# mikestir/webradio

Measured on AMD Instinct MI355X. Metric: complex Msamples/sec (node), 256-ch DDC+NFM demod, higher is better.
Workload: dtype f32

## Files before the change

include/webradio_amd.h:

```cpp
#ifndef WEBRADIO_AMD_H_
#define WEBRADIO_AMD_H_

#include <stddef.h>
#include <stdint.h>

#ifdef __cplusplus
extern "C" {
#endif

#define WR_ABI_VERSION   6
#define WR_FIR_LENGTH    64
#define WR_TABLE_SIZE    65536

enum wr_status {
	WR_OK = 0,
	WR_ERR_ARG = 1,
	WR_ERR_HIP = 2,
	WR_ERR_STATE = 3,
	WR_ERR_NOMEM = 4,
	WR_ERR_NODEV = 5,
	WR_ERR_RATE = 6
};

enum wr_mode { WR_AM = 0, WR_FM = 1, WR_USB = 2, WR_LSB = 3 };
// ... 128 lines not shown
int wr_tuner_mark_launches(wr_tuner *tuner, int enable);
int wr_ring_exchange_after(wr_ring *ring, wr_tuner *tuner, const float *send_dev, float *recv_dev, size_t nfloats);
int wr_ring_wait(wr_ring *ring);
int wr_ring_info(wr_ring *ring, int *rank, int *world, unsigned long long *exchanges);
int wr_ring_destroy(wr_ring *ring);
int wr_tuner_set_audio_scale(wr_tuner *tuner, float scale);

int wr_tuner_set_blocks_per_launch(wr_tuner *tuner, unsigned int nblocks);

#define WR_STREAM_MAX_BLOCKS 512u
int wr_tuner_set_streaming(wr_tuner *tuner, int enable);
int wr_tuner_stream_info(wr_tuner *tuner, int *live, unsigned long long *launches, unsigned long long *blocks);
int wr_tuner_stream_host_blocks(wr_tuner *tuner, unsigned long long *blocks);
int wr_tuner_stream_long_blocks(wr_tuner *tuner, unsigned long long *blocks);

int wr_tuner_profile(wr_tuner *tuner, int enable);
int wr_tuner_profile_read(wr_tuner *tuner, unsigned int *launches, double *mean_ms);

int wr_spectrum_create(wr_spectrum **spec, wr_dev *dev, unsigned int fft_size, unsigned int hop);
int wr_spectrum_create_real(wr_spectrum **spec, wr_dev *dev, unsigned int fft_size, unsigned int hop);
int wr_spectrum_channels(wr_spectrum *spec, unsigned int *channels);
int wr_spectrum_destroy(wr_spectrum *spec);
int wr_spectrum_push(wr_spectrum *spec, const float *iq, size_t nframes, int where);
int wr_spectrum_lazy_info(wr_spectrum *spec, unsigned long long *deferred_pushes, unsigned long long *resolves);
int wr_spectrum_get_db(wr_spectrum *spec, float *magnitudes_host );
int wr_spectrum_get_bins(wr_spectrum *spec, float *bins_host );
int wr_spectrum_frames_done(wr_spectrum *spec, unsigned long *frames);
int wr_spectrum_get_waterfall_row(wr_spectrum *spec, unsigned int width, int hold,
                                  float *db_row_host, uint8_t *palette_host);
int wr_spectrum_batch_db(wr_spectrum *spec, const float *iq_dev, size_t nframes_fft,
// ... 9 lines not shown
```

webradio_amd/capi.py:

```python
import ctypes as C
import os

_HERE = os.path.dirname(os.path.abspath(__file__))
LIB_PATH = os.path.join(_HERE, "lib", "libwebradio_amd.so")

WR_OK, WR_ERR_ARG, WR_ERR_HIP, WR_ERR_STATE, WR_ERR_NOMEM, WR_ERR_NODEV, WR_ERR_RATE = range(7)
WR_AM, WR_FM, WR_USB, WR_LSB = range(4)
WR_STAGE_CHAN_IQ, WR_STAGE_DEMOD, WR_STAGE_AUDIO = 1, 2, 3
WR_NCO_SPLIT, WR_NCO_EXACT, WR_NCO_ROTATE = 0, 1, 2
WR_HOST, WR_DEVICE = 0, 1
WR_ABI_VERSION = 6
WR_STREAM_MAX_BLOCKS = 512
WR_FIR_LENGTH = 64
WR_TABLE_SIZE = 65536

_fp = C.POINTER(C.c_float)
_vp = C.c_void_p
_u32 = C.c_uint
_sz = C.c_size_t

SIGNATURES = {
    "wr_abi_version": (C.c_int, []),
    "wr_last_error": (C.c_char_p, []),
    "wr_device_count": (C.c_int, [C.POINTER(C.c_int)]),
# ... 32 lines not shown
    "wr_chan_set_if": (C.c_int, [_vp, C.c_int, C.c_int]),
    "wr_chan_set_filter": (C.c_int, [_vp, C.c_int, C.c_int, _u32, _u32]),
    "wr_chan_set_taps": (C.c_int, [_vp, C.c_int, C.c_int, _vp, _u32]),
    "wr_chan_set_filter_n": (C.c_int, [_vp, C.c_int, C.c_int, _u32, _u32, _u32]),
    "wr_chan_set_taps_n": (C.c_int, [_vp, C.c_int, C.c_int, _vp, _u32, _u32]),
    "wr_chan_set_mode": (C.c_int, [_vp, C.c_int, C.c_int]),
    "wr_chan_set_af_gain": (C.c_int, [_vp, C.c_int, C.c_float]),
    "wr_chan_set_squelch": (C.c_int, [_vp, C.c_int, C.c_float, C.c_int]),
    "wr_tuner_keep_stages": (C.c_int, [_vp, _u32]),
    "wr_tuner_flush": (C.c_int, [_vp]),
    "wr_tuner_set_blocks_per_launch": (C.c_int, [_vp, _u32]),
    "wr_tuner_set_streaming": (C.c_int, [_vp, C.c_int]),
    "wr_tuner_stream_info": (C.c_int, [_vp, C.POINTER(C.c_int), C.POINTER(C.c_ulonglong), C.POINTER(C.c_ulonglong)]),
    "wr_tuner_stream_host_blocks": (C.c_int, [_vp, C.POINTER(C.c_ulonglong)]),
    "wr_tuner_stream_long_blocks": (C.c_int, [_vp, C.POINTER(C.c_ulonglong)]),
    "wr_tuner_seek": (C.c_int, [_vp, C.c_ulonglong]),
    "wr_tuner_audio_ring": (C.c_int, [_vp, _u32]),
    "wr_tuner_audio_ring_acquire": (C.c_int, [_vp, C.POINTER(C.POINTER(C.c_float)), C.POINTER(C.c_size_t),
                                              C.POINTER(C.c_size_t), C.POINTER(_u32), C.POINTER(C.c_ulonglong)]),
    "wr_tuner_audio_ring_release": (C.c_int, [_vp]),
    "wr_tuner_audio_ring_ready": (C.c_int, [_vp, C.POINTER(C.c_int)]),
    "wr_tuner_audio_ring_stats": (C.c_int, [_vp, C.POINTER(_u32), C.POINTER(C.c_ulonglong)]),
    "wr_tuner_submit_count": (C.c_int, [_vp, C.POINTER(C.c_ulonglong)]),
    "wr_chan_get_state": (C.c_int, [_vp, C.c_int, C.POINTER(_u32), _vp]),
    "wr_chan_set_state": (C.c_int, [_vp, C.c_int, _u32, _vp]),
    "wr_tuner_submit": (C.c_int, [_vp, _vp, _sz, C.c_int]),
    "wr_tuner_last_staging": (C.c_int, [_vp, C.POINTER(C.c_int)]),
    "wr_block_kernel_calls": (C.c_ulonglong, []),
    "wr_tuner_submit_u8": (C.c_int, [_vp, _vp, _sz, C.c_int]),
    "wr_chan_fetch": (C.c_int, [_vp, C.c_int, C.c_int, _vp, _sz, C.POINTER(_sz)]),
# ... 77 lines not shown
```

webradio_amd/csrc/wr_capi_internal.h:

```cpp
#ifndef WR_CAPI_INTERNAL_H
#define WR_CAPI_INTERNAL_H

#include "wr_internal.h"

#include <cstdarg>
#include <cstdio>
#include <cstdlib>
#include <cstring>
#include <new>
#include <atomic>
#include <chrono>
#include <map>
#include <mutex>
#include <vector>

#define HIP_TRY(expr)                                                                    \
	do {                                                                                 \
		hipError_t e_ = (expr);                                                          \
		if (e_ != hipSuccess)                                                            \
			return wrc_fail(WR_ERR_HIP, "%s: %s (%s:%d)", #expr, hipGetErrorString(e_),  \
			                __FILE__, __LINE__);                                         \
	} while (0)


// ... 72 lines not shown
	bool seek_pending = false;
	unsigned long long seek_frame = 0;
	float *z_hist = nullptr, *z_prev = nullptr, *z_dem = nullptr;
	bool pend_direct = false;
	unsigned long long pend_seq = 0;
	size_t pend_k2 = 0;
	unsigned int pend_slots = 0;
	int sp;
	int cb;
	int last_cb;
	std::vector<int> owner;
	bool dirty;
	bool uniform_taps;
	unsigned long long uniform_mask = 0;
	unsigned long long uniform2_mask = 0;
	unsigned long long fewsets_mask = 0;
	unsigned char nsets[64] = {0};
	bool one_filter = false;
	bool long_uniform = false;
	bool long_one = false;
	size_t last_k1, last_k2;
	int active;
};

struct wr_tuner {
	wr_dev *dev;
	unsigned int input_rate;
	unsigned int max_channels;
	size_t max_block_frames;
	int nco_mode;
// ... 46 lines not shown
		bool host_bytes = false;
		bool live = false;
		bool unchecked = false;
		WrStreamCtl *ctl = nullptr;
		WrStreamDesc *desc = nullptr;
		WrStreamDev *sdev = nullptr;
		float *ring = nullptr;
		size_t ring_floats = 0;
		Group *g = nullptr;
		unsigned int count = 0;
		size_t nframes = 0;
		bool u8 = false;
		int parity0 = 0;
		size_t k1 = 0, k2 = 0;
		unsigned long long gen = 0;
		unsigned long long blocks = 0;
		std::chrono::steady_clock::time_point last_bell;
		const float *last_iq = nullptr;
		uint8_t *raw[4] = {nullptr, nullptr, nullptr, nullptr};
		size_t raw_cap = 0;
		unsigned long long raw_next = 0;
		unsigned long long raw_gen[4] = {0, 0, 0, 0};
		unsigned int raw_idx[4] = {0, 0, 0, 0};
		hipEvent_t raw_ev = nullptr;
		bool ext = false;
		bool up_pending = false;
		unsigned long long host_blocks = 0;
		unsigned long long long_blocks = 0;
	} stream;
};
// ... 65 lines not shown
```

webradio_amd/csrc/wr_internal.h:

```cpp
#ifndef WR_INTERNAL_H_
#define WR_INTERNAL_H_

#include <hip/hip_runtime.h>
#include <stddef.h>
#include <stdint.h>

#include "webradio_amd.h"

#define WR_HIST      (WR_FIR_LENGTH - 1)
#define WR_LANES     64
#define WR_SPLIT_N   256
#define WR_MAX_DEVICES 64
#define WR_TAPSETS   4

int         wrc_fail(int code, const char *fmt, ...) __attribute__((format(printf, 2, 3)));
int         wrc_dev_index(const wr_dev *dev);
hipStream_t wrc_dev_stream(const wr_dev *dev);
int         wrc_tuner_launch_mark(wr_tuner *t, hipEvent_t *ev);

void     wrd_sin_table(float *table);
void     wrd_sin_table_rounded(float *table);
int      wrd_phase_step(int if_hz, unsigned int input_rate);
unsigned wrd_lowpass_maxbin(unsigned int fir_length, unsigned int passband, unsigned int input_rate);
void     wrd_lowpass_design(unsigned int fir_length, unsigned int passband, unsigned int input_rate, float *coeff);
// ... 36 lines not shown
	float       *hist_next;
	int          parity;
	int          sp;
	int          cb;
	size_t       nframes;
	unsigned int d1, d2;
	unsigned int slots;
	unsigned int slots_used;
	size_t       k1, k2;
	size_t       k2max;
	int          nco_mode;
	float        audio_scale;
	int          use_gain, use_squelch;
	unsigned long long uniform_mask;
	unsigned long long uniform2_mask;
	unsigned long long fewsets_mask;
	unsigned char nsets[64];
	int          one_filter;
	void        *ev_start, *ev_stop;
	bool         seeking = false;
	unsigned int seek_lo = 0;
};

hipError_t wrk_mix(hipStream_t st, const float *in, float *out, size_t nframes,
                   unsigned int phase, int step, const float *table_dev);
hipError_t wrk_fir(hipStream_t st, const float *in, size_t nframes, unsigned int channels,
                   unsigned int decim, unsigned int fir_length, const float *coeff_dev, const float *hist_dev,
                   float *out);
hipError_t wrk_hist_update(hipStream_t st, const float *in, size_t nframes, unsigned int channels,
                           unsigned int fir_length, float *hist_dev, float *scratch_dev);
// ... 6 lines not shown
struct WrPostArgs {
	const float *chan_iq;
	unsigned int k1, slots;
	const int   *mode;
	const float *prev_iq;
	float       *prev_next;
	const float *dem_hist;
	float       *dem_hist_next;
	size_t       k2;
	unsigned int tiles;
	unsigned int run;
	unsigned int ntiles;
	const float *taps2;
	const float *taps2u;
	unsigned long long uni2;
	float       *audio;
	size_t       k2max;
	float        scale;
	unsigned int d2;
	unsigned int groups;
	const float *gain;
	const float *squelch;
	float       *audio_host;
	size_t       host_stride;
	unsigned int nseg = 1;
	const float *chan_prev = nullptr;
};
long wrk_tune_ng2_min_passes(long value, bool set);
hipError_t wrk_tuner_ddc(hipStream_t st, const WrTunerLaunch &L, const WrGroupDev &G,
                         const float *table_dev, const float *hi_dev, const float *lo_dev,
// ... 114 lines not shown
```

webradio_amd/csrc/wr_kernels.hip:

```cpp
#include "wr_internal.h"

#include <atomic>
#include <cstdlib>
#include <type_traits>

#include <hip/hip_ext.h>

typedef float v2f __attribute__((ext_vector_type(2)));
typedef __attribute__((address_space(3))) v2f lds_v2f;
typedef float v4f __attribute__((ext_vector_type(4)));
typedef __attribute__((address_space(3))) v4f lds_v4f;

#define PHASE_FLAG_ACTIVE   1

#define WR_CONSTANT __attribute__((address_space(4)))

#ifdef DDC_TIMELINE
#define TL_SLOTS 12
__device__ unsigned long long g_ddc_tl[16384 * TL_SLOTS];
extern "C" int wr_debug_timeline(unsigned long long *out, size_t n)
{
	return (int)hipMemcpyFromSymbol(out, HIP_SYMBOL(g_ddc_tl), n * sizeof(unsigned long long));
}
__device__ unsigned long long g_ddc_rt[16384 * 2];
// ... 337 lines not shown
		if (!chan_prev)
			return dem_hist[rr * slots + s];
		const size_t kp = (size_t)k1 - hist + rr;
		const float2 z = chan_prev[kp * slots + s];
		const float2 zp = chan_prev[(kp - 1u) * slots + s];
		return demod_one(m, z.x, z.y, zp.x, zp.y);
	}
	const size_t kk = rr - hist;
	if (kk >= k1)
		return 0.0f;
	const float2 z = chan_iq[kk * slots + s];
	const float2 zp = kk ? chan_iq[(kk - 1u) * slots + s] : chan_prev ? chan_prev[((size_t)k1 - 1u) * slots + s] : prev_iq[s];
	return demod_one(m, z.x, z.y, zp.x, zp.y);
}

template <unsigned int D2, bool HREGS, unsigned int NSEG = 1u>
__device__ __forceinline__ void post_role(const WrPostArgs &A, unsigned int bx, unsigned int g,
                                          float *stage, float *tile, int *modes)
{
	constexpr unsigned int HIST = WR_FIR_LENGTH * NSEG - 1u;
	constexpr unsigned int NEED = (POST_TK - 1u) * D2 + WR_FIR_LENGTH * NSEG;
	constexpr unsigned int NROW = POST_THREADS / 64u;
	static_assert(NSEG == 1u || !HREGS, "the segmented filter reads its taps when their turn comes (measured at C2, 128 / 256 taps: "
	                                    "61 / 83 us per block; a segment's 64 taps fetched into registers first: 64 / 94)");
	const float2 *__restrict__ chan_iq = (const float2 *)A.chan_iq;
	const float2 *__restrict__ prev_iq = (const float2 *)A.prev_iq;
	const float2 *__restrict__ chan_prev = (const float2 *)A.chan_prev;
	const float *__restrict__ dem_hist = A.dem_hist;
	const float *__restrict__ taps2 = A.taps2;
	const unsigned int k1 = A.k1, slots = A.slots;
	const unsigned int lane = threadIdx.x & 63u;
	const unsigned int row = threadIdx.x >> 6;
	const unsigned int s = g * 64u + lane;
	const int m = A.mode[s];

	if (bx == A.ntiles) {
		if (m < 0)
			return;
		const size_t first = k1;
#pragma unroll
		for (unsigned int r = row; r < HIST; r += NROW)
			A.dem_hist_next[(size_t)r * slots + s] = post_row(chan_iq, k1, slots, s, m, prev_iq, dem_hist, first + r, chan_prev, HIST);
		if (row == 0)
			((float2 *)A.prev_next)[s] = k1 ? chan_iq[(size_t)(k1 - 1u) * slots + s] : prev_iq[s];
		return;
	}

	TLP(0);
	float h[HREGS ? WR_FIR_LENGTH : 1];
	if (HREGS && row < POST_TK / POST_B) {
#pragma unroll
		for (int j = 0; j < (HREGS ? WR_FIR_LENGTH : 1); ++j)
			h[j] = taps2[(size_t)j * slots + s];
	}
	if (row == 0)
		modes[lane] = m;
	constexpr unsigned int FRESH = POST_TK * D2;
// ... 16 lines not shown
			__syncthreads();
#pragma unroll
			for (unsigned int i = 0; i < CARRY_PER; ++i) {
				const unsigned int e = threadIdx.x + i * POST_THREADS;
				if (e < CARRY * 64u)
					stage[e] = keep[i];
			}
			first = CARRY;
		}
		{
			const unsigned int per = (NEED - first + NROW - 1u) / NROW;
			const unsigned int beg = first + row * per;
			const unsigned int end = (beg + per < NEED) ? beg + per : NEED;
			if (r0 > HIST && r0 + NEED <= (size_t)k1 + HIST) {
				const float2 *__restrict__ src = chan_iq + (r0 - HIST) * slots + s;
				for (unsigned int r = beg; r < end; r += POST_LB) {
					float2 z[POST_LB + 1u];
					z[0] = src[((size_t)r - 1u) * slots];
#pragma unroll
					for (unsigned int i = 0; i < POST_LB; ++i) {
						const unsigned int ri = (r + i < end) ? r + i : end - 1u;
						z[i + 1u] = src[(size_t)ri * slots];
					}
#pragma unroll
					for (unsigned int i = 0; i < POST_LB; ++i)
						if (r + i < end)
							stage[(r + i) * 64u + lane] = (m >= 0) ? demod_one(m, z[i + 1u].x, z[i + 1u].y, z[i].x, z[i].y) : 0.0f;
				}
			} else {
				float2 zp = make_float2(0.0f, 0.0f);
				if (m >= 0 && beg < end) {
					const size_t rr = r0 + beg;
					if (rr == HIST)
						zp = chan_prev ? chan_prev[((size_t)k1 - 1u) * slots + s] : prev_iq[s];
					else if (rr > HIST && rr - HIST - 1u < k1)
						zp = chan_iq[(rr - HIST - 1u) * slots + s];
					else if (rr < HIST && chan_prev)
						zp = chan_prev[((size_t)k1 - HIST - 1u + rr) * slots + s];
				}
#pragma unroll 6
				for (unsigned int r = beg; r < end; ++r) {
					const size_t rr = r0 + r;
					float v = 0.0f;
					if (m >= 0) {
						if (rr < HIST && chan_prev) {
							const float2 z = chan_prev[((size_t)k1 - HIST + rr) * slots + s];
							v = demod_one(m, z.x, z.y, zp.x, zp.y);
							zp = z;
						} else if (rr < HIST) {
							v = dem_hist[rr * slots + s];
							if (rr + 1u == HIST)
								zp = prev_iq[s];
						} else if (rr - HIST < k1) {
							const float2 z = chan_iq[(rr - HIST) * slots + s];
							v = demod_one(m, z.x, z.y, zp.x, zp.y);
							zp = z;
						}
					}
					stage[r * 64u + lane] = v;
				}
			}
		}
		__syncthreads();
		TLP(1);
		if (row < POST_TK / POST_B) {
			float acc[POST_B];
#pragma unroll
			for (unsigned int o = 0; o < POST_B; ++o)
				acc[o] = 0.0f;
// ... 1707 lines not shown
	A.mode = G.mode;
	A.prev_iq = G.prev_iq[p];
	A.prev_next = G.prev_iq[p ^ 1];
	A.dem_hist = G.dem[p];
	A.dem_hist_next = G.dem[p ^ 1];
	A.k2 = L.k2;
	A.tiles = (unsigned int)((L.k2 + POST_TK - 1) / POST_TK);
	{
		const unsigned int all = A.tiles * (L.slots_used / 64u);
		A.run = all >= 1536u ? 4u : all >= 384u ? 2u : 1u;
	}
	A.ntiles = (A.tiles + A.run - 1u) / A.run;
	A.taps2 = G.taps2;
	A.taps2u = G.taps2u;
	A.uni2 = L.uniform2_mask;
	A.audio = G.audio;
	A.k2max = L.k2max;
	A.scale = L.audio_scale;
	A.d2 = L.d2;
	A.groups = L.slots_used / 64;
	A.gain = L.use_gain ? G.gain : nullptr;
	A.squelch = L.use_squelch ? G.squelch : nullptr;
	A.audio_host = nullptr;
	A.host_stride = 0;
	A.nseg = G.l2 / WR_FIR_LENGTH;
	return A;
}

template <unsigned int D2>
static hipError_t launch_post(hipStream_t st, const WrPostArgs &A)
// ... 133 lines not shown
```

webradio_amd/csrc/wr_stream_kernel.inc:

```

__device__ __forceinline__ unsigned int st_rfl(unsigned int v) { return __builtin_amdgcn_readfirstlane(v); }
__device__ __forceinline__ unsigned int st_ld(const unsigned int *p)
{
	return st_rfl(__hip_atomic_load(p, __ATOMIC_RELAXED, __HIP_MEMORY_SCOPE_AGENT));
}
__device__ __forceinline__ unsigned long long st_ld64(const unsigned long long *p)
{
	const unsigned long long v = __hip_atomic_load(p, __ATOMIC_RELAXED, __HIP_MEMORY_SCOPE_AGENT);
	return ((unsigned long long)st_rfl((unsigned int)(v >> 32)) << 32) | st_rfl((unsigned int)v);
}
__device__ __forceinline__ unsigned int st_ld_sys(const volatile unsigned int *p)
{
	return st_rfl(__hip_atomic_load((const unsigned int *)p, __ATOMIC_RELAXED, __HIP_MEMORY_SCOPE_SYSTEM));
}
__device__ __forceinline__ void st_st_sys(volatile unsigned int *p, unsigned int v)
{
	__hip_atomic_store((unsigned int *)p, v, __ATOMIC_RELAXED, __HIP_MEMORY_SCOPE_SYSTEM);
}

__device__ __forceinline__ unsigned int st_ddc_ready(const WrStreamArgs &S)
{
	return st_rfl((unsigned int)__hip_atomic_load(&S.sdev->progress, __ATOMIC_RELAXED, __HIP_MEMORY_SCOPE_AGENT));
}
__device__ __forceinline__ unsigned int st_post_ready(const WrStreamArgs &S)
// ... 199 lines not shown
			asm volatile("s_waitcnt vmcnt(0)" ::: "memory");
			__hip_atomic_store(&S.sdev->stop, 1u, __ATOMIC_RELAXED, __HIP_MEMORY_SCOPE_AGENT);
			return;
		}
		if (seen >= WR_STREAM_MAXJ || __builtin_amdgcn_s_memrealtime() - t_last > S.idle_ticks) {
			if (seen < WR_STREAM_MAXJ)
				st_st_sys(&S.ctl->self_closed, 1u);
			asm volatile("s_waitcnt vmcnt(0)" ::: "memory");
			__hip_atomic_store(&S.sdev->stop, 1u, __ATOMIC_RELAXED, __HIP_MEMORY_SCOPE_AGENT);
			return;
		}
		__builtin_amdgcn_s_sleep(40);
	}
}

template <unsigned int PD2, unsigned int TS, unsigned int NSEG>
__device__ __forceinline__ void stream_post(const WrStreamArgs &S, const unsigned int p, v2f *lds, const bool helper)
{
	constexpr unsigned int D2 = PD2 ? PD2 : 1u;
	constexpr unsigned int NEED = (POST_TK - 1u) * D2 + WR_FIR_LENGTH * NSEG;
	wave_prio(3u);
	if (threadIdx.x >= POST_THREADS)
		return;
	const unsigned int wave = st_rfl(threadIdx.x >> 6);
	const unsigned int waves_per_wg = POST_THREADS / 64u;
#ifdef STREAM_TL
	if (threadIdx.x == 0 && S.tl && !helper)
		S.tl[(6000u + p) * 8u + 7u] = 12345ull;
#endif

	const unsigned int n_bnd = (S.kslow * S.groups + waves_per_wg - 1u) / waves_per_wg;
	if (!helper && p < n_bnd) {
		const unsigned long long c0 = S.cur0;
		ddc_body<WR_NCO_ROTATE, true, PD2>(S.is_u8 ? nullptr : (const float2 *)c0, S.is_u8 ? (const uchar2 *)c0 : nullptr,
		                                   (const float2 *)S.hist, (float2 *)S.hist_next, (size_t)S.nframes, (size_t)S.k1, S.d1,
		                                   S.slots, S.groups, S.phase, S.step, (const float2 *)S.hist_cs, S.flags, S.phase_next,
		                                   (float2 *)S.hist_cs_next, (const float2 *)S.hist_lo, (float2 *)S.hist_lo_next, S.taps1,
		                                   (const float4 *)S.rot, S.taps1u, S.tapsel, TS == 1u ? 1u : S.kmax, (float2 *)S.ring, S.table,
		                                   (const float2 *)S.hi_cs, (const float2 *)S.lo_cs, S.n_ddc, S.post, S.gmap0, S.gmap1, 0,
		                                   S.kslow, 0x40000000u, 0u, 0u, lds, DDC_ROLE_BOUNDARY);
		const unsigned int ub = p * waves_per_wg + wave;
		asm volatile("s_waitcnt vmcnt(0)" ::: "memory");
		if (ub / S.groups < S.kslow && (threadIdx.x & 63u) == 0u)
			__hip_atomic_fetch_add(&S.sdev->ddc_done[0][ub % WR_STREAM_SHARDS][0], 1u, __ATOMIC_RELAXED, __HIP_MEMORY_SCOPE_AGENT);
		wave_prio(3u);
		__syncthreads();
	}

	float *stage = (float *)lds;
// ... 84 lines not shown
			A.run = S.drain_run;
			A.ntiles = S.drain_ntiles;
		}
		const unsigned int tasks_j = A.ntiles * A.groups;
		unsigned int mine = 0;
		const unsigned int rot = (unsigned int)(((unsigned long long)j * tasks) % S.n_post);
		for (unsigned int t = p >= rot ? p - rot : p + S.n_post - rot;; t += S.n_post) {
			if (drain) {
				if (threadIdx.x == 0)
					sh[4] = __hip_atomic_fetch_add(&S.sdev->post_ticket[j], 1u, __ATOMIC_RELAXED, __HIP_MEMORY_SCOPE_AGENT);
				__syncthreads();
				t = sh[4];
			}
			if (t >= tasks_j)
				break;
			post_role<D2, false, NSEG>(A, t % A.ntiles, t / A.ntiles, stage, tile, modes);
			__syncthreads();
			++mine;
		}
		if (threadIdx.x == 0 && mine) {
			if (ah)
				__builtin_amdgcn_fence(__ATOMIC_RELEASE, "");
			else
				__builtin_amdgcn_fence(__ATOMIC_RELEASE, "agent");
			asm volatile("s_waitcnt vmcnt(0)" ::: "memory");
			__hip_atomic_fetch_add(&S.sdev->post_done[j], mine, __ATOMIC_RELAXED, __HIP_MEMORY_SCOPE_AGENT);
		}
#ifdef STREAM_TL
		if (threadIdx.x == 0 && S.tl && !helper && p < 4u && j < 256u)
			S.tl[(7300u + j) * 8u + p * 2u + 1u] = __builtin_amdgcn_s_memrealtime();
		if (threadIdx.x == 0) {
// ... 8 lines not shown
	if (threadIdx.x == 0 && S.tl && !helper) {
		S.tl[(6000u + p) * 8u + 0u] = pt_wait;
		S.tl[(6000u + p) * 8u + 1u] = pt_sync;
		S.tl[(6000u + p) * 8u + 2u] = pt_n;
	}
#endif
	if (!helper && p < S.post.groups && known && known <= WR_STREAM_MAXJ) {
		const unsigned int jl = known - 1u;
		WrPostArgs A = S.post;
		A.chan_iq = S.ring + (size_t)(jl % WR_STREAM_RING) * S.k1 * S.slots * 2u;
		A.chan_prev = jl ? S.ring + (size_t)((jl - 1u) % WR_STREAM_RING) * S.k1 * S.slots * 2u : nullptr;
		A.prev_iq = S.prev_iq[S.parity0];
		A.dem_hist = S.dem[S.parity0];
		A.prev_next = const_cast<float *>(S.prev_iq[S.parity0 ^ 1]);
		A.dem_hist_next = S.dem[S.parity0 ^ 1];
		post_role<D2, false, NSEG>(A, A.ntiles, p, stage, tile, modes);
	}
}

template <unsigned int NG, unsigned int TS>
__device__ __forceinline__ void stream_ddc(const WrStreamArgs &S, v2f *lds)
{
	static_assert(TS == 1u || (TS == WR_TAPSETS && NG == 1u), "several channel filters: one lane group per wave");
	constexpr int NCO = WR_NCO_ROTATE;
	const unsigned int lane = threadIdx.x & 63u;
	const unsigned int wave = st_rfl(threadIdx.x >> 6);
	const unsigned int waves_per_wg = blockDim.x >> 6;
	const unsigned int wid = blockIdx.x * waves_per_wg + wave;
	wave_prio(3u);
	rot_tables_to_lds(lds, (const float2 *)S.hi_cs, (const float2 *)S.lo_cs);
	const v2f *hi_l = lds, *lo_l = lds + WR_SPLIT_N;
// ... 240 lines not shown
				const unsigned int b = __hip_atomic_load((const unsigned short *)c + n, __ATOMIC_RELAXED, __HIP_MEMORY_SCOPE_AGENT);
				v = make_float2(((float)(b & 255u) - 128.0f) / 128.0f, ((float)(b >> 8) - 128.0f) / 128.0f);
			} else if (S.ext) {
				const unsigned long long x = __hip_atomic_load((const unsigned long long *)c + n, __ATOMIC_RELAXED, __HIP_MEMORY_SCOPE_AGENT);
				v = make_float2(__builtin_bit_cast(float, (unsigned int)x), __builtin_bit_cast(float, (unsigned int)(x >> 32)));
			} else {
				v = input_frame(S.is_u8 ? nullptr : (const float2 *)c, S.is_u8 ? (const uchar2 *)c : nullptr, n);
			}
			((float2 *)S.hist_next)[lane] = v;
		}
		if (lane == 0)
			st_st_sys(&S.ctl->final_blocks, known);
	}
}

template <unsigned int PD2, unsigned int NG, unsigned int TS, unsigned int NSEG>
__global__ void __launch_bounds__(DDC_ROTATE_WAVES * 64u) __attribute__((amdgpu_waves_per_eu(DDC_NG2_WAVES_PER_EU)))
k_tuner_stream(const WrStreamArgs S)
{
	extern __shared__ v2f lds[];
	if (blockIdx.x >= S.n_ddc + S.n_post) {
		stream_bell(S);
		return;
	}
	const bool ddc = blockIdx.x < S.n_ddc;
	if (ddc) {
		stream_ddc<NG, TS>(S, lds);
		__syncthreads();
	}
	stream_post<PD2, TS, NSEG>(S, ddc ? blockIdx.x : blockIdx.x - S.n_ddc, lds, ddc);
}

static unsigned int stream_post_run(unsigned int tiles, unsigned int groups, unsigned int max_post)
{
	unsigned int run = 1;
	while (run < tiles && ((tiles + run - 1u) / run) * groups > max_post)
		++run;
	return run;
}

static size_t stream_lds_bytes(unsigned int d2, unsigned int nset, unsigned int nseg)
{
	const size_t post_lds = post_lds_bytes(d2, nseg) + 16u * sizeof(float);
	const size_t ddc_lds = (size_t)DDC_ROTATE_WAVES * 2u * 512u * nset + 2u * WR_SPLIT_N * 8u;
	return post_lds > ddc_lds ? post_lds : ddc_lds;
// ... 23 lines not shown
	return hipErrorInvalidValue;
}

template <unsigned int PD2, unsigned int NG, unsigned int TS, unsigned int NSEG>
static hipError_t stream_allow_lds(size_t lds)
{
	static bool attr_done[WR_MAX_DEVICES];
	if (lds <= 64 * 1024)
		return hipSuccess;
	return allow_lds((const void *)k_tuner_stream<PD2, NG, TS, NSEG>, stream_lds_bytes(PD2, TS, NSEG), attr_done);
}

template <unsigned int PD2, unsigned int NG, unsigned int TS, unsigned int NSEG>
static hipError_t stream_occupancy(size_t lds, int *per_cu)
{
	hipError_t e = stream_allow_lds<PD2, NG, TS, NSEG>(lds);
	if (e != hipSuccess)
		return e;
	return hipOccupancyMaxActiveBlocksPerMultiprocessor(per_cu, k_tuner_stream<PD2, NG, TS, NSEG>, (int)(DDC_ROTATE_WAVES * 64u), lds);
}

hipError_t wrk_stream_geometry(unsigned int d2, unsigned int groups, unsigned int kmax, bool one_filter, unsigned int nseg,
                               int num_cus, unsigned int *n_ddc, unsigned int *n_post)
{
	*n_ddc = *n_post = 0;
	if (!wrk_tuner_post_supported(d2) || !stream_nseg_supported(d2, nseg) || !groups || groups > 16u || !kmax ||
	    kmax > WR_TAPSETS)
		return hipSuccess;
	unsigned int ng, ts;
	stream_shape(groups, kmax, one_filter, &ng, &ts);
	const size_t lds = stream_lds_bytes(d2, ts == 1u ? 1u : kmax, nseg);
	int per_cu = 0;
	hipError_t e = with_post_d2(d2, [&](auto D2) {
		constexpr unsigned int PD2 = decltype(D2)::value;
		return with_stream_nseg<PD2>(nseg, [&](auto NS) {
			constexpr unsigned int NSEG = decltype(NS)::value;
			return ts != 1u ? stream_occupancy<PD2, 1, WR_TAPSETS, NSEG>(lds, &per_cu)
			       : ng == 1u ? stream_occupancy<PD2, 1, 1, NSEG>(lds, &per_cu)
			                  : stream_occupancy<PD2, 2, 1, NSEG>(lds, &per_cu);
		});
	});
	if (e != hipSuccess)
		return e;
	if (per_cu > 3)
		per_cu = 3;
	if (per_cu < 2)
		return hipSuccess;
	*n_ddc = (unsigned int)(per_cu - 1) * (unsigned int)num_cus;
	*n_post = (unsigned int)num_cus - 4u;
	return hipSuccess;
}

template <unsigned int PD2, unsigned int NG, unsigned int TS, unsigned int NSEG>
static hipError_t launch_stream(hipStream_t st, const WrStreamArgs &A, void *ev_start, void *ev_stop)
{
	const size_t lds = stream_lds_bytes(PD2, TS == 1u ? 1u : A.kmax, NSEG);
	hipError_t e = stream_allow_lds<PD2, NG, TS, NSEG>(lds);
	if (e != hipSuccess)
		return e;
	const unsigned int grid = A.n_ddc + A.n_post + 1u;
// ... 46 lines not shown
```

webradio_amd/csrc/wr_tuner.hip:

```cpp
#include "wr_capi_internal.h"

static int dev_alloc_zero(void **p, size_t count, size_t elem)
{
	HIP_TRY(hipMalloc(p, (count ? count : 1) * elem));
	HIP_TRY(hipMemset(*p, 0, (count ? count : 1) * elem));
	HIP_TRY(hipStreamSynchronize(nullptr));
	return WR_OK;
}


unsigned int wrc_group_slots_used(const Group *g)
{
	unsigned int hi = 0;
	for (unsigned int s = 0; s < g->slots; ++s)
		if (g->owner[s] >= 0)
			hi = s + 1;
	return ((hi + WR_LANES - 1) / WR_LANES) * WR_LANES;
}

WrTunerLaunch wrc_group_launch(const wr_tuner *t, const Group *g, const float *cur, const uint8_t *cur_u8,
                               size_t nframes)
{
	WrTunerLaunch L;
	L.cur = cur;
// ... 2 lines not shown
	L.hist_next = t->in_hist[t->in_par ^ 1];
	L.parity = g->parity;
	L.sp = g->sp;
	L.cb = g->cb;
	L.nframes = nframes;
	L.d1 = g->d1;
	L.d2 = g->d2;
	L.slots = g->slots;
	L.slots_used = wrc_group_slots_used(g);
	L.k1 = nframes / g->d1;
	L.k2 = L.k1 / g->d2;
	L.k2max = g->k2max;
	L.nco_mode = t->nco_mode;
	L.uniform_mask = g->uniform_mask;
	L.uniform2_mask = g->uniform2_mask;
	L.fewsets_mask = g->fewsets_mask;
	L.one_filter = g->one_filter ? 1 : 0;
	memcpy(L.nsets, g->nsets, sizeof(L.nsets));
	L.audio_scale = t->audio_scale;
	L.use_gain = g->use_gain ? 1 : 0;
	L.use_squelch = g->use_squelch ? 1 : 0;
	L.ev_start = L.ev_stop = nullptr;
	return L;
}

struct GroupArray {
	void **p;
	size_t count, elem;
};
static std::vector<GroupArray> group_arrays(Group *g)
// ... 724 lines not shown
		for (int j = 0; j < WR_FIR_LENGTH; ++j)
			taps1[(size_t)j * S + s] = c.taps[0][j];
		for (unsigned int j = 0; j < g->l2; ++j)
			taps2[(size_t)j * S + s] = g->l2 > WR_FIR_LENGTH ? c.taps_long2[j] : c.taps[1][j];
		if (g->d1b)
			for (unsigned int j = 0; j < g->l1b; ++j)
				taps1b[(size_t)j * S + s] = g->l1b > WR_FIR_LENGTH ? c.taps_long1b[j] : c.taps[2][j];
		if (g->l1 > WR_FIR_LENGTH)
			for (unsigned int j = 0; j < g->l1; ++j)
				taps1L[(size_t)j * S + s] = c.taps_long[j];
		gain[s] = c.gain;
		squelch[s] = c.squelch;
		g->use_gain = g->use_gain || c.gain != 1.0f;
		g->use_squelch = g->use_squelch || c.squelch > 0.0f;
	}
	GroupFilters F;
	group_classify(t, g, F);
	std::vector<float> rot(S * 4, 0.0f);
	{
		const float *turn = t->dev->turn_host;
		for (size_t s = 0; s < S; ++s) {
			const unsigned int Sx = step[s] >> 16;
			rot[4 * s + 0] = turn[(Sx + 16384u) & 0xFFFFu];
			rot[4 * s + 1] = turn[Sx & 0xFFFFu];
			rot[4 * s + 2] = turn[(Sx + 16385u) & 0xFFFFu];
			rot[4 * s + 3] = turn[(Sx + 1u) & 0xFFFFu];
		}
	}
	HIP_TRY(hipMemcpyAsync(g->dev.step, step.data(), S * sizeof(unsigned int), hipMemcpyHostToDevice, st));
	HIP_TRY(hipMemcpyAsync(g->dev.flags, flags.data(), S * sizeof(int), hipMemcpyHostToDevice, st));
// ... 746 lines not shown
```

webradio_amd/csrc/wr_tuner_stream.hip:

```cpp
#include "wr_capi_internal.h"


static unsigned long long *g_stream_tl = nullptr;
extern "C" int wr_debug_stream_tl(unsigned long long *out, size_t n)
{
	if (!g_stream_tl)
		return 1;
	memcpy(out, g_stream_tl, n * sizeof(unsigned long long));
	return 0;
}

static std::mutex g_stream_mu;
static wr_tuner *g_stream_on[WR_MAX_DEVICES];

static void stream_raw_free(wr_tuner::Stream &s)
{
	for (uint8_t *&r : s.raw) {
		(void)hipFree(r);
		r = nullptr;
	}
	s.raw_cap = 0;
}

void wrc_stream_free(wr_tuner *t)
// ... 139 lines not shown
	HIP_TRY(hipHostGetDevicePointer(&ctl_dev, s.ctl, 0));
	HIP_TRY(hipHostGetDevicePointer(&desc_dev, s.desc, 0));
	hipStream_t st = d->stream;

	const WrTunerLaunch L = wrc_group_launch(t, g, u8 ? nullptr : (const float *)iq, u8 ? (const uint8_t *)iq : nullptr, nframes);

	WrStreamArgs A;
	memset(&A, 0, sizeof(A));
	A.ctl = (WrStreamCtl *)ctl_dev;
	A.desc_host = (const WrStreamDesc *)desc_dev;
	A.sdev = s.sdev;
	A.idle_ticks = (unsigned long long)WR_STREAM_IDLE_MS * 100000ull;
	A.wait_ticks = (unsigned long long)WR_STREAM_WAIT_MS * 100000ull;
	A.n_ddc = n_ddc;
	A.n_post = n_post;
	if (getenv("WR_STREAM_TL") && atoi(getenv("WR_STREAM_TL"))) {
		static unsigned long long *tlbuf = nullptr;
		if (!tlbuf)
			HIP_TRY(hipHostMalloc((void **)&tlbuf, 8192 * 8 * sizeof(unsigned long long), hipHostMallocMapped | hipHostMallocCoherent));
		memset(tlbuf, 0, 8192 * 8 * sizeof(unsigned long long));
		void *tld = nullptr;
		HIP_TRY(hipHostGetDevicePointer(&tld, tlbuf, 0));
		A.tl = (unsigned long long *)tld;
		g_stream_tl = tlbuf;
	}
	A.nframes = nframes;
	A.k1 = (unsigned int)k1;
	A.d1 = g->d1;
	A.is_u8 = u8 ? 1u : 0u;
	A.ext = s.ext ? 1u : 0u;
// ... 217 lines not shown
}

extern "C" int wr_tuner_stream_info(wr_tuner *t, int *live, unsigned long long *launches, unsigned long long *blocks)
{
	if (!t)
		return wrc_fail(WR_ERR_ARG, "tuner is NULL");
	if (live)
		*live = t->stream.live ? 1 : 0;
	if (launches)
		*launches = t->stream.gen;
	if (blocks)
		*blocks = t->stream.blocks;
	return WR_OK;
}

extern "C" int wr_tuner_stream_long_blocks(wr_tuner *t, unsigned long long *blocks)
{
	if (!t || !blocks)
		return wrc_fail(WR_ERR_ARG, "wr_tuner_stream_long_blocks: bad argument");
	*blocks = t->stream.long_blocks;
	return WR_OK;
}

extern "C" int wr_tuner_stream_host_blocks(wr_tuner *t, unsigned long long *blocks)
{
	if (!t || !blocks)
		return wrc_fail(WR_ERR_ARG, "wr_tuner_stream_host_blocks: bad argument");
	*blocks = t->stream.host_blocks;
	return WR_OK;
}
// ... 1 lines not shown
```

webradio_amd/device.py:

```python
import ctypes as C

import numpy as np

from . import capi
from .capi import check, ptr


class Device:

    def __init__(self, index=0, stream=None):
        self.lib = capi.load()
        h = C.c_void_p()
        check(self.lib.wr_dev_open(C.byref(h), index, ptr(stream) if stream else None))
        self.h = h
        self.index = index

    def close(self):
        if self.h:
            self.lib.wr_dev_close(self.h)
            self.h = None

    def sync(self):
        check(self.lib.wr_dev_sync(self.h))

# ... 97 lines not shown
        check(self.lib.wr_tuner_set_blocks_per_launch(self.h, n))

    def streaming(self, enable=True):
        check(self.lib.wr_tuner_set_streaming(self.h, int(enable) if enable is not True else 1))

    def stream_info(self):
        live, launches, blocks = C.c_int(), C.c_ulonglong(), C.c_ulonglong()
        check(self.lib.wr_tuner_stream_info(self.h, C.byref(live), C.byref(launches), C.byref(blocks)))
        return bool(live.value), launches.value, blocks.value

    def stream_host_blocks(self):
        n = C.c_ulonglong()
        check(self.lib.wr_tuner_stream_host_blocks(self.h, C.byref(n)))
        return n.value

    def stream_long_blocks(self):
        n = C.c_ulonglong()
        check(self.lib.wr_tuner_stream_long_blocks(self.h, C.byref(n)))
        return n.value

    def mark_launches(self, enable=True):
        check(self.lib.wr_tuner_mark_launches(self.h, 1 if enable else 0))

    def seek(self, frame):
        check(self.lib.wr_tuner_seek(self.h, C.c_ulonglong(frame)))

    def fetch_audio_all(self):
        stride, frames, slots = C.c_size_t(), C.c_size_t(), C.c_uint()
        self.lib.wr_tuner_fetch_audio_all(self.h, None, 0, C.byref(stride), C.byref(frames), C.byref(slots))
        out = np.empty(max(1, slots.value * frames.value), dtype=np.float32)
# ... 207 lines not shown
```

Baseline: 119,200.

## Raise streaming kernel occupancy to four blocks per CU with lean post path

When the post stage's LDS footprint allows it (NG=2, TS=1, NSEG=1), the persistent streaming kernel now asks for 8 waves per EU and allows four resident blocks per CU instead of the fixed cap of three. To fit the tighter register budget, the post role gets a LEAN variant: smaller unroll factors, a rolled history loop, and a fast path for wave-sized channel groups that all use the same demod mode, dispatched once through readfirstlane into a mode-specialised row loop. A host-computed unimode mask marks those groups. The PD2 template argument to the boundary DDC body is forced to zero, and a geometry query API is added. More resident blocks give more DDC workers and latency hiding, at the cost of register pressure and possible spills.

```diff
diff --git a/include/webradio_amd.h b/include/webradio_amd.h
--- a/include/webradio_amd.h
+++ b/include/webradio_amd.h
@@ -166,6 +166,8 @@
 int wr_tuner_stream_host_blocks(wr_tuner *tuner, unsigned long long *blocks);
 int wr_tuner_stream_long_blocks(wr_tuner *tuner, unsigned long long *blocks);
 
+int wr_tuner_stream_geometry(wr_tuner *tuner, unsigned int *n_ddc, unsigned int *n_post);
+
 int wr_tuner_profile(wr_tuner *tuner, int enable);
 int wr_tuner_profile_read(wr_tuner *tuner, unsigned int *launches, double *mean_ms);
 
diff --git a/webradio_amd/capi.py b/webradio_amd/capi.py
--- a/webradio_amd/capi.py
+++ b/webradio_amd/capi.py
@@ -70,6 +70,7 @@
     "wr_tuner_stream_info": (C.c_int, [_vp, C.POINTER(C.c_int), C.POINTER(C.c_ulonglong), C.POINTER(C.c_ulonglong)]),
     "wr_tuner_stream_host_blocks": (C.c_int, [_vp, C.POINTER(C.c_ulonglong)]),
     "wr_tuner_stream_long_blocks": (C.c_int, [_vp, C.POINTER(C.c_ulonglong)]),
+    "wr_tuner_stream_geometry": (C.c_int, [_vp, C.POINTER(_u32), C.POINTER(_u32)]),
     "wr_tuner_seek": (C.c_int, [_vp, C.c_ulonglong]),
     "wr_tuner_audio_ring": (C.c_int, [_vp, _u32]),
     "wr_tuner_audio_ring_acquire": (C.c_int, [_vp, C.POINTER(C.POINTER(C.c_float)), C.POINTER(C.c_size_t),
diff --git a/webradio_amd/csrc/wr_capi_internal.h b/webradio_amd/csrc/wr_capi_internal.h
--- a/webradio_amd/csrc/wr_capi_internal.h
+++ b/webradio_amd/csrc/wr_capi_internal.h
@@ -110,6 +110,7 @@
 	bool uniform_taps;
 	unsigned long long uniform_mask = 0;
 	unsigned long long uniform2_mask = 0;
+	unsigned long long unimode_mask = 0;
 	unsigned long long fewsets_mask = 0;
 	unsigned char nsets[64] = {0};
 	bool one_filter = false;
@@ -186,6 +187,7 @@
 		int parity0 = 0;
 		size_t k1 = 0, k2 = 0;
 		unsigned long long gen = 0;
+		unsigned int n_ddc = 0, n_post = 0;
 		unsigned long long blocks = 0;
 		std::chrono::steady_clock::time_point last_bell;
 		const float *last_iq = nullptr;
diff --git a/webradio_amd/csrc/wr_internal.h b/webradio_amd/csrc/wr_internal.h
--- a/webradio_amd/csrc/wr_internal.h
+++ b/webradio_amd/csrc/wr_internal.h
@@ -74,6 +74,7 @@
 	int          use_gain, use_squelch;
 	unsigned long long uniform_mask;
 	unsigned long long uniform2_mask;
+	unsigned long long unimode_mask;
 	unsigned long long fewsets_mask;
 	unsigned char nsets[64];
 	int          one_filter;
@@ -110,6 +111,7 @@
 	const float *taps2;
 	const float *taps2u;
 	unsigned long long uni2;
+	unsigned long long unim;
 	float       *audio;
 	size_t       k2max;
 	float        scale;
diff --git a/webradio_amd/csrc/wr_kernels.hip b/webradio_amd/csrc/wr_kernels.hip
--- a/webradio_amd/csrc/wr_kernels.hip
+++ b/webradio_amd/csrc/wr_kernels.hip
@@ -375,7 +375,38 @@
 	return demod_one(m, z.x, z.y, zp.x, zp.y);
 }
 
-template <unsigned int D2, bool HREGS, unsigned int NSEG = 1u>
+template <int MODE>
+__device__ __forceinline__ void post_rows_uniform(const float2 *__restrict__ p, size_t stride, float *st, unsigned int n)
+{
+	float2 zp = *p;
+	p += stride;
+	unsigned int r = 0;
+	for (; r + POST_LB <= n; r += POST_LB) {
+		float2 z[POST_LB];
+#pragma unroll
+		for (unsigned int i = 0; i < POST_LB; ++i) {
+			z[i] = *p;
+			p += stride;
+		}
+		asm volatile("s_waitcnt vmcnt(0)" ::: "memory");
+#pragma unroll
+		for (unsigned int i = 0; i < POST_LB; ++i) {
+			const float2 q = i ? z[i - 1u] : zp;
+			st[i * 64u] = demod_one(MODE, z[i].x, z[i].y, q.x, q.y);
+		}
+		zp = z[POST_LB - 1u];
+		st += POST_LB * 64u;
+	}
+	for (; r < n; ++r) {
+		const float2 z = *p;
+		p += stride;
+		*st = demod_one(MODE, z.x, z.y, zp.x, zp.y);
+		zp = z;
+		st += 64u;
+	}
+}
+
+template <unsigned int D2, bool HREGS, unsigned int NSEG = 1u, bool LEAN = false>
 __device__ __forceinline__ void post_role(const WrPostArgs &A, unsigned int bx, unsigned int g,
                                           float *stage, float *tile, int *modes)
 {
@@ -399,9 +430,15 @@
 		if (m < 0)
 			return;
 		const size_t first = k1;
+		if constexpr (LEAN) {
+#pragma unroll 1
+			for (unsigned int r = row; r < HIST; r += NROW)
+				A.dem_hist_next[(size_t)r * slots + s] = post_row(chan_iq, k1, slots, s, m, prev_iq, dem_hist, first + r, chan_prev, HIST);
+		} else {
 #pragma unroll
 		for (unsigned int r = row; r < HIST; r += NROW)
 			A.dem_hist_next[(size_t)r * slots + s] = post_row(chan_iq, k1, slots, s, m, prev_iq, dem_hist, first + r, chan_prev, HIST);
+		}
 		if (row == 0)
 			((float2 *)A.prev_next)[s] = k1 ? chan_iq[(size_t)(k1 - 1u) * slots + s] : prev_iq[s];
 		return;
@@ -448,20 +485,34 @@
 			const unsigned int end = (beg + per < NEED) ? beg + per : NEED;
 			if (r0 > HIST && r0 + NEED <= (size_t)k1 + HIST) {
 				const float2 *__restrict__ src = chan_iq + (r0 - HIST) * slots + s;
-				for (unsigned int r = beg; r < end; r += POST_LB) {
-					float2 z[POST_LB + 1u];
+				constexpr unsigned int LB = LEAN ? 2u : POST_LB;
+				if (LEAN && g < 64u && ((A.unim >> g) & 1ull)) {
+					if (beg < end) {
+						const float2 *__restrict__ p = src + ((size_t)beg - 1u) * slots;
+						float *st = stage + beg * 64u + lane;
+						switch (__builtin_amdgcn_readfirstlane(m)) {
+						case WR_AM: post_rows_uniform<WR_AM>(p, slots, st, end - beg); break;
+						case WR_FM: post_rows_uniform<WR_FM>(p, slots, st, end - beg); break;
+						case WR_USB: post_rows_uniform<WR_USB>(p, slots, st, end - beg); break;
+						default: post_rows_uniform<WR_LSB>(p, slots, st, end - beg); break;
+						}
+					}
+				} else
+				for (unsigned int r = beg; r < end; r += LB) {
+					float2 z[LB + 1u];
 					z[0] = src[((size_t)r - 1u) * slots];
 #pragma unroll
-					for (unsigned int i = 0; i < POST_LB; ++i) {
+					for (unsigned int i = 0; i < LB; ++i) {
 						const unsigned int ri = (r + i < end) ? r + i : end - 1u;
 						z[i + 1u] = src[(size_t)ri * slots];
 					}
 #pragma unroll
-					for (unsigned int i = 0; i < POST_LB; ++i)
+					for (unsigned int i = 0; i < LB; ++i)
 						if (r + i < end)
 							stage[(r + i) * 64u + lane] = (m >= 0) ? demod_one(m, z[i + 1u].x, z[i + 1u].y, z[i].x, z[i].y) : 0.0f;
 				}
 			} else {
+				constexpr unsigned int SLOW_UNROLL = LEAN ? 1u : 6u;
 				float2 zp = make_float2(0.0f, 0.0f);
 				if (m >= 0 && beg < end) {
 					const size_t rr = r0 + beg;
@@ -472,21 +523,18 @@
 					else if (rr < HIST && chan_prev)
 						zp = chan_prev[((size_t)k1 - HIST - 1u + rr) * slots + s];
 				}
-#pragma unroll 6
+#pragma unroll SLOW_UNROLL
 				for (unsigned int r = beg; r < end; ++r) {
 					const size_t rr = r0 + r;
 					float v = 0.0f;
 					if (m >= 0) {
-						if (rr < HIST && chan_prev) {
-							const float2 z = chan_prev[((size_t)k1 - HIST + rr) * slots + s];
-							v = demod_one(m, z.x, z.y, zp.x, zp.y);
-							zp = z;
-						} else if (rr < HIST) {
+						const bool hprev = rr < HIST && chan_prev;
+						if (rr < HIST && !hprev) {
 							v = dem_hist[rr * slots + s];
 							if (rr + 1u == HIST)
 								zp = prev_iq[s];
-						} else if (rr - HIST < k1) {
-							const float2 z = chan_iq[(rr - HIST) * slots + s];
+						} else if (hprev || rr - HIST < k1) {
+							const float2 z = hprev ? chan_prev[((size_t)k1 - HIST + rr) * slots + s] : chan_iq[(rr - HIST) * slots + s];
 							v = demod_one(m, z.x, z.y, zp.x, zp.y);
 							zp = z;
 						}
@@ -2224,6 +2272,7 @@
 	A.taps2 = G.taps2;
 	A.taps2u = G.taps2u;
 	A.uni2 = L.uniform2_mask;
+	A.unim = L.unimode_mask;
 	A.audio = G.audio;
 	A.k2max = L.k2max;
 	A.scale = L.audio_scale;
diff --git a/webradio_amd/csrc/wr_stream_kernel.inc b/webradio_amd/csrc/wr_stream_kernel.inc
--- a/webradio_amd/csrc/wr_stream_kernel.inc
+++ b/webradio_amd/csrc/wr_stream_kernel.inc
@@ -237,7 +237,7 @@
 	}
 }
 
-template <unsigned int PD2, unsigned int TS, unsigned int NSEG>
+template <unsigned int PD2, unsigned int TS, unsigned int NSEG, bool LEAN>
 __device__ __forceinline__ void stream_post(const WrStreamArgs &S, const unsigned int p, v2f *lds, const bool helper)
 {
 	constexpr unsigned int D2 = PD2 ? PD2 : 1u;
@@ -255,7 +255,7 @@
 	const unsigned int n_bnd = (S.kslow * S.groups + waves_per_wg - 1u) / waves_per_wg;
 	if (!helper && p < n_bnd) {
 		const unsigned long long c0 = S.cur0;
-		ddc_body<WR_NCO_ROTATE, true, PD2>(S.is_u8 ? nullptr : (const float2 *)c0, S.is_u8 ? (const uchar2 *)c0 : nullptr,
+		ddc_body<WR_NCO_ROTATE, true, 0u>(S.is_u8 ? nullptr : (const float2 *)c0, S.is_u8 ? (const uchar2 *)c0 : nullptr,
 		                                   (const float2 *)S.hist, (float2 *)S.hist_next, (size_t)S.nframes, (size_t)S.k1, S.d1,
 		                                   S.slots, S.groups, S.phase, S.step, (const float2 *)S.hist_cs, S.flags, S.phase_next,
 		                                   (float2 *)S.hist_cs_next, (const float2 *)S.hist_lo, (float2 *)S.hist_lo_next, S.taps1,
@@ -370,7 +370,7 @@
 			}
 			if (t >= tasks_j)
 				break;
-			post_role<D2, false, NSEG>(A, t % A.ntiles, t / A.ntiles, stage, tile, modes);
+			post_role<D2, false, NSEG, LEAN>(A, t % A.ntiles, t / A.ntiles, stage, tile, modes);
 			__syncthreads();
 			++mine;
 		}
@@ -409,7 +409,7 @@
 		A.dem_hist = S.dem[S.parity0];
 		A.prev_next = const_cast<float *>(S.prev_iq[S.parity0 ^ 1]);
 		A.dem_hist_next = S.dem[S.parity0 ^ 1];
-		post_role<D2, false, NSEG>(A, A.ntiles, p, stage, tile, modes);
+		post_role<D2, false, NSEG, LEAN>(A, A.ntiles, p, stage, tile, modes);
 	}
 }
 
@@ -680,8 +680,16 @@
 	}
 }
 
+#define STREAM_LDS_PER_CU (160u * 1024u)
+template <unsigned int PD2, unsigned int NG, unsigned int TS, unsigned int NSEG> struct StreamOcc {
+	static constexpr size_t post_lds = (((size_t)(POST_TK - 1u) * (PD2 ? PD2 : 1u) + WR_FIR_LENGTH * NSEG) * 64u + POST_TK * 65u + 64u + 16u) * sizeof(float);
+	static constexpr bool four = NG == 2u && TS == 1u && NSEG == 1u && 4u * post_lds <= STREAM_LDS_PER_CU;
+	static constexpr unsigned int per_eu = four ? 8u : DDC_NG2_WAVES_PER_EU;
+	static constexpr int per_cu = four ? 4 : 3;
+};
+
 template <unsigned int PD2, unsigned int NG, unsigned int TS, unsigned int NSEG>
-__global__ void __launch_bounds__(DDC_ROTATE_WAVES * 64u) __attribute__((amdgpu_waves_per_eu(DDC_NG2_WAVES_PER_EU)))
+__global__ void __launch_bounds__(DDC_ROTATE_WAVES * 64u) __attribute__((amdgpu_waves_per_eu(StreamOcc<PD2, NG, TS, NSEG>::per_eu)))
 k_tuner_stream(const WrStreamArgs S)
 {
 	extern __shared__ v2f lds[];
@@ -694,7 +702,7 @@
 		stream_ddc<NG, TS>(S, lds);
 		__syncthreads();
 	}
-	stream_post<PD2, TS, NSEG>(S, ddc ? blockIdx.x : blockIdx.x - S.n_ddc, lds, ddc);
+	stream_post<PD2, TS, NSEG, StreamOcc<PD2, NG, TS, NSEG>::four>(S, ddc ? blockIdx.x : blockIdx.x - S.n_ddc, lds, ddc);
 }
 
 static unsigned int stream_post_run(unsigned int tiles, unsigned int groups, unsigned int max_post)
@@ -748,10 +756,15 @@
 template <unsigned int PD2, unsigned int NG, unsigned int TS, unsigned int NSEG>
 static hipError_t stream_occupancy(size_t lds, int *per_cu)
 {
+	static_assert(!StreamOcc<PD2, NG, TS, NSEG>::four || StreamOcc<PD2, NG, TS, NSEG>::post_lds >= (size_t)DDC_ROTATE_WAVES * 2u * 512u + 2u * WR_SPLIT_N * 8u,
+	              "StreamOcc counts the post stage's LDS: it must be the larger one");
 	hipError_t e = stream_allow_lds<PD2, NG, TS, NSEG>(lds);
 	if (e != hipSuccess)
 		return e;
-	return hipOccupancyMaxActiveBlocksPerMultiprocessor(per_cu, k_tuner_stream<PD2, NG, TS, NSEG>, (int)(DDC_ROTATE_WAVES * 64u), lds);
+	e = hipOccupancyMaxActiveBlocksPerMultiprocessor(per_cu, k_tuner_stream<PD2, NG, TS, NSEG>, (int)(DDC_ROTATE_WAVES * 64u), lds);
+	if (e == hipSuccess && *per_cu > StreamOcc<PD2, NG, TS, NSEG>::per_cu)
+		*per_cu = StreamOcc<PD2, NG, TS, NSEG>::per_cu;
+	return e;
 }
 
 hipError_t wrk_stream_geometry(unsigned int d2, unsigned int groups, unsigned int kmax, bool one_filter, unsigned int nseg,
@@ -776,8 +789,6 @@
 	});
 	if (e != hipSuccess)
 		return e;
-	if (per_cu > 3)
-		per_cu = 3;
 	if (per_cu < 2)
 		return hipSuccess;
 	*n_ddc = (unsigned int)(per_cu - 1) * (unsigned int)num_cus;
diff --git a/webradio_amd/csrc/wr_tuner.hip b/webradio_amd/csrc/wr_tuner.hip
--- a/webradio_amd/csrc/wr_tuner.hip
+++ b/webradio_amd/csrc/wr_tuner.hip
@@ -40,6 +40,7 @@
 	L.nco_mode = t->nco_mode;
 	L.uniform_mask = g->uniform_mask;
 	L.uniform2_mask = g->uniform2_mask;
+	L.unimode_mask = g->unimode_mask;
 	L.fewsets_mask = g->fewsets_mask;
 	L.one_filter = g->one_filter ? 1 : 0;
 	memcpy(L.nsets, g->nsets, sizeof(L.nsets));
@@ -794,6 +795,14 @@
 		g->use_gain = g->use_gain || c.gain != 1.0f;
 		g->use_squelch = g->use_squelch || c.squelch > 0.0f;
 	}
+	g->unimode_mask = 0;
+	for (size_t base = 0; base + WR_LANES <= S && base / WR_LANES < 64; base += WR_LANES) {
+		bool same = mode[base] >= 0;
+		for (size_t s = base + 1; s < base + WR_LANES && same; ++s)
+			same = mode[s] == mode[base];
+		if (same)
+			g->unimode_mask |= 1ull << (base / WR_LANES);
+	}
 	GroupFilters F;
 	group_classify(t, g, F);
 	std::vector<float> rot(S * 4, 0.0f);
diff --git a/webradio_amd/csrc/wr_tuner_stream.hip b/webradio_amd/csrc/wr_tuner_stream.hip
--- a/webradio_amd/csrc/wr_tuner_stream.hip
+++ b/webradio_amd/csrc/wr_tuner_stream.hip
@@ -177,6 +177,8 @@
 	A.wait_ticks = (unsigned long long)WR_STREAM_WAIT_MS * 100000ull;
 	A.n_ddc = n_ddc;
 	A.n_post = n_post;
+	s.n_ddc = n_ddc;
+	s.n_post = n_post;
 	if (getenv("WR_STREAM_TL") && atoi(getenv("WR_STREAM_TL"))) {
 		static unsigned long long *tlbuf = nullptr;
 		if (!tlbuf)
@@ -424,6 +426,17 @@
 	return WR_OK;
 }
 
+extern "C" int wr_tuner_stream_geometry(wr_tuner *t, unsigned int *n_ddc, unsigned int *n_post)
+{
+	if (!t)
+		return wrc_fail(WR_ERR_ARG, "tuner is NULL");
+	if (n_ddc)
+		*n_ddc = t->stream.n_ddc;
+	if (n_post)
+		*n_post = t->stream.n_post;
+	return WR_OK;
+}
+
 extern "C" int wr_tuner_stream_long_blocks(wr_tuner *t, unsigned long long *blocks)
 {
 	if (!t || !blocks)
diff --git a/webradio_amd/device.py b/webradio_amd/device.py
--- a/webradio_amd/device.py
+++ b/webradio_amd/device.py
@@ -135,6 +135,11 @@
         check(self.lib.wr_tuner_stream_host_blocks(self.h, C.byref(n)))
         return n.value
 
+    def stream_geometry(self):
+        a, b = C.c_uint32(), C.c_uint32()
+        check(self.lib.wr_tuner_stream_geometry(self.h, C.byref(a), C.byref(b)))
+        return a.value, b.value
+
     def stream_long_blocks(self):
         n = C.c_ulonglong()
         check(self.lib.wr_tuner_stream_long_blocks(self.h, C.byref(n)))
```

Result: slower. 110,600 (-7.2%).
